# Rongjiehuang/FastDiff

Measured on AMD Instinct MI355X. Metric: real-time factor (audio-sec/wall-sec), N=4 reverse steps, 80x864 mel, higher is better.
Workload: dtype f32 results; 2-piece fp16 operands (22 bit) on fp16 MFMA, fp32 accumulate; GEMM as Winograd F(2,3); exact-fp32 twin; 1 GPU; BASELINE configs[1]: LJSpeech shape, batch=8 x 80x864 mel per GPU, N=4, HIP kernels + hipGraph sampler; batch_per_gpu=8, frames=864, reverse_steps=4, graph=True, weights=random init seed 1234 (no checkpoint offline), world_size=1, gpus_visible=1, oversubscribed=False

## Files before the change

### fastdiff_amd/csrc/fd_kernels_common.h

```cpp
#ifndef FD_KERNELS_COMMON_H
#define FD_KERNELS_COMMON_H
#include "fd_kernels.h"
#include "fd_device.h"

typedef float f32x16 __attribute__((ext_vector_type(16)));

namespace fdk_fast {

__device__ __forceinline__ f32x16 mfma32(float a, float b, f32x16 c)
{
    return __builtin_amdgcn_mfma_f32_32x32x2f32(a, b, c, 0, 0, 0);
}
__device__ __forceinline__ int drow(int r, int hi) { return (r & 3) + 8 * (r >> 2) + 4 * hi; }
__device__ __forceinline__ int opaque(int x)
{
    asm volatile("" : "+v"(x));
    return x;
}
__device__ __forceinline__ float lrelu(float v, float s)
{
    return __builtin_amdgcn_fmed3f(v, v * s, __builtin_inff());
}
__device__ __forceinline__ float f4c(const float4 &v, int r) { return r == 0 ? v.x : (r == 1 ? v.y : (r == 2 ? v.z : v.w)); }

__device__ __forceinline__ int frames_of(const int *lens, int b, int T) { return lens ? lens[b] : T; }

__device__ __forceinline__ bool skip_after_previous_overflow(int *flag)
{
    if (flag[32] == 0) return false;
    if (blockIdx.x == 0 && blockIdx.y == 0 && blockIdx.z == 0 && threadIdx.x == 0) atomicOr(flag, 1);
    return true;
}

constexpr float GX_SCALE = 2048.0f, GX_INV_SCALE = 1.0f / 2048.0f;
constexpr float GX_LIMIT = 32768.0f;
typedef _Float16 f16x8 __attribute__((ext_vector_type(8)));
__device__ __forceinline__ f32x16 mfma_f16(const float4 &a, const float4 &b, f32x16 c)
{
    union { float4 f; f16x8 h; } ua, ub;
    ua.f = a;
    ub.f = b;
    return __builtin_amdgcn_mfma_f32_32x32x16_f16(ua.h, ub.h, c, 0, 0, 0);
}

typedef _Float16 h2_t __attribute__((ext_vector_type(2)));
typedef float f2_t __attribute__((ext_vector_type(2)));

__device__ __forceinline__ void split2(float a, float b, unsigned &hi, unsigned &lo)
{
    const f2_t v = {a, b};
    const h2_t h = __builtin_convertvector(v, h2_t);
    const f2_t r = (v - __builtin_convertvector(h, f2_t)) * GX_SCALE;
    const h2_t l = __builtin_convertvector(r, h2_t);
    hi = __builtin_bit_cast(unsigned, h);
    lo = __builtin_bit_cast(unsigned, l);
}
__device__ __forceinline__ void split8(const float (&v)[8], float4 &hi, float4 &lo)
{
    unsigned h[4], l[4];
#pragma unroll
    for (int i = 0; i < 4; ++i) split2(v[2 * i], v[2 * i + 1], h[i], l[i]);
    hi = make_float4(__uint_as_float(h[0]), __uint_as_float(h[1]), __uint_as_float(h[2]), __uint_as_float(h[3]));
    lo = make_float4(__uint_as_float(l[0]), __uint_as_float(l[1]), __uint_as_float(l[2]), __uint_as_float(l[3]));
}
__device__ __forceinline__ float amax4(float m, const float4 &v) { return fmaxf(fmaxf(m, fmaxf(fabsf(v.x), fabsf(v.y))), fmaxf(fabsf(v.z), fabsf(v.w))); }
__device__ __forceinline__ int h2_off(int row, int slot) { return row * 128 + ((slot ^ ((row >> 1) & 7)) << 4); }
__device__ __forceinline__ void halo_dot(const char *xs, int row, int slot, const float4 &w1f, const float4 &w2f, float &a1, float &a2)
{
    union { float4 f; h2_t h[4]; } x1, x2, w1, w2;
    x1.f = *reinterpret_cast<const float4 *>(xs + h2_off(row, slot));
    x2.f = *reinterpret_cast<const float4 *>(xs + h2_off(row, 4 + slot));
    w1.f = w1f;
    w2.f = w2f;
#pragma unroll
    for (int q = 0; q < 4; ++q) {
        a1 = __builtin_amdgcn_fdot2(w1.h[q], x1.h[q], a1, false);
        a2 = __builtin_amdgcn_fdot2(w1.h[q], x2.h[q], a2, false);
        a2 = __builtin_amdgcn_fdot2(w2.h[q], x1.h[q], a2, false);
    }
}


#ifndef FD_LVC_NT
#define FD_LVC_NT 66
#endif
typedef float lvc_f4 __attribute__((ext_vector_type(4)));
template <int BIT>
__device__ __forceinline__ float4 lvc_ld(const float4 *p)
{
    if constexpr ((FD_LVC_NT & BIT) != 0) {
        const lvc_f4 v = __builtin_nontemporal_load(reinterpret_cast<const lvc_f4 *>(p));
        return make_float4(v.x, v.y, v.z, v.w);
    } else return *p;
}
template <int BIT>
__device__ __forceinline__ void lvc_st(float *p, float v) { if constexpr ((FD_LVC_NT & BIT) != 0) __builtin_nontemporal_store(v, p); else *p = v; }
template <int BIT>
__device__ __forceinline__ void lvc_st(float4 *p, const float4 &v)
{
    if constexpr ((FD_LVC_NT & BIT) != 0) __builtin_nontemporal_store(lvc_f4{v.x, v.y, v.z, v.w}, reinterpret_cast<lvc_f4 *>(p));
    else *p = v;
}

#ifndef FD_LVC_XCD_RUN
#define FD_LVC_XCD_RUN 8
#endif
template <int R = FD_LVC_XCD_RUN>
__device__ __forceinline__ int lvc_tile_of_workgroup()
{
    constexpr int G = 8 * R;
    const int n = blockIdx.x;
    if constexpr (R <= 1) return n;
    const int g0 = (n / G) * G;
    return (g0 + G <= (int)gridDim.x) ? g0 + (n % 8) * R + (n / 8) % R : n;
}

}
#endif
```

### fastdiff_amd/csrc/fd_kernels_dblock.hip

```cpp
#include "fd_kernels_common.h"

namespace fdk_fast {

constexpr int DB_LD = 136;
constexpr int DB_STRIDE = 114;

template <int DIL, bool LRELU>
__device__ __forceinline__ void conv96_tile(f32x16 &acc, const float4 (&wa)[12], const float *in, int ld, int col, int hi)
{
    const int o[3] = {opaque(hi * ld + col - DIL), opaque(hi * ld + col), opaque(hi * ld + col + DIL)};
#pragma unroll
    for (int s = 0; s < 48; ++s) {
        const int tap = s >> 4, c2 = (2 * s) & 31;
        float v = in[o[tap] + c2 * ld];
        if (LRELU) v = lrelu(v, 0.2f);
        acc = mfma32(f4c(wa[s >> 2], s & 3), v, acc);
    }
}

template <int F>
__global__ void __launch_bounds__(256, 2) k_dblock(const float *__restrict__ xin, float *__restrict__ out,
                                                   const float *__restrict__ p0, const float *__restrict__ p1,
                                                   const float *__restrict__ p2, const float *__restrict__ pr,
                                                   const float *__restrict__ b0, const float *__restrict__ b1,
                                                   const float *__restrict__ b2, const float *__restrict__ br, int Lin, int Lo,
                                                   const int *__restrict__ run_if, const int *__restrict__ lens, int per_frame)
{
    __shared__ __attribute__((aligned(16))) float xs[fd::C * DB_LD];
    if (run_if && *run_if == 0) return;
    __shared__ __attribute__((aligned(16))) float hA[fd::C * DB_LD];
    __shared__ __attribute__((aligned(16))) float hB[fd::C * DB_LD];
    const int b = blockIdx.y, tid = threadIdx.x, lane = tid & 63, wave = tid >> 6, l31 = lane & 31, hi = lane >> 5;
    const int pbase = blockIdx.x * DB_STRIDE - 7;
    const int Lob = lens ? lens[b] * per_frame : Lo;
    if (blockIdx.x * DB_STRIDE >= Lob) return;
    {
        constexpr int NK = fd::C * DB_LD / 256;
        float v[NK];
#pragma unroll
        for (int k = 0; k < NK; ++k) {
            const int idx = k * 256 + tid, ci = idx / DB_LD, cc = idx - ci * DB_LD, p = pbase + cc - 4;
            v[k] = (cc >= 4 && cc < 132 && p >= 0 && p < Lob) ? xin[((int64_t)b * fd::C + ci) * Lin + (int64_t)p * F] : 0.0f;
        }
#pragma unroll
        for (int k = 0; k < NK; ++k) {
            const int idx = k * 256 + tid;
            xs[idx] = v[k];
            hA[idx] = 0.0f;
            hB[idx] = 0.0f;
        }
    }
    __syncthreads();
    const int c = wave * 32 + l31;
    const int p = pbase + c;
    const bool inside = (p >= 0 && p < Lob);
    float4 wa[12];
    f32x16 acc;
#pragma unroll
    for (int i = 0; i < 12; ++i) wa[i] = reinterpret_cast<const float4 *>(p0)[i * 64 + lane];
#pragma unroll
    for (int r = 0; r < 16; ++r) acc[r] = b0[drow(r, hi)];
    conv96_tile<1, true>(acc, wa, xs, DB_LD, 4 + c, hi);
#pragma unroll
    for (int r = 0; r < 16; ++r) hA[drow(r, hi) * DB_LD + 4 + c] = inside ? acc[r] : 0.0f;
    __syncthreads();
#pragma unroll
    for (int i = 0; i < 12; ++i) wa[i] = reinterpret_cast<const float4 *>(p1)[i * 64 + lane];
#pragma unroll
    for (int r = 0; r < 16; ++r) acc[r] = b1[drow(r, hi)];
    conv96_tile<2, true>(acc, wa, hA, DB_LD, 4 + c, hi);
#pragma unroll
    for (int r = 0; r < 16; ++r) hB[drow(r, hi) * DB_LD + 4 + c] = inside ? acc[r] : 0.0f;
    __syncthreads();
#pragma unroll
    for (int i = 0; i < 12; ++i) wa[i] = reinterpret_cast<const float4 *>(p2)[i * 64 + lane];
#pragma unroll
    for (int r = 0; r < 16; ++r) acc[r] = b2[drow(r, hi)] + br[drow(r, hi)];
    conv96_tile<4, true>(acc, wa, hB, DB_LD, 4 + c, hi);
    {
        float4 wr[4];
#pragma unroll
        for (int i = 0; i < 4; ++i) wr[i] = reinterpret_cast<const float4 *>(pr)[i * 64 + lane];
#pragma unroll
        for (int s = 0; s < 16; ++s) acc = mfma32(f4c(wr[s >> 2], s & 3), xs[(2 * s + hi) * DB_LD + 4 + c], acc);
    }
    if (inside && c >= 7 && c < 7 + DB_STRIDE) {
#pragma unroll
        for (int r = 0; r < 16; ++r) out[((int64_t)b * fd::C + drow(r, hi)) * Lo + p] = acc[r];
    }
}

constexpr int DBH_ROWS = 136;

template <int DIL>
__device__ __forceinline__ void conv96_h2(f32x16 &ah, f32x16 &al, const float4 (&wa)[2][6], const char *img, int c, int hi)
{
    int off[3][2][2];
#pragma unroll
    for (int tap = 0; tap < 3; ++tap)
#pragma unroll
        for (int p = 0; p < 2; ++p)
#pragma unroll
            for (int c2 = 0; c2 < 2; ++c2) off[tap][p][c2] = h2_off(4 + c + (tap - 1) * DIL, p * 4 + c2 * 2 + hi);
#pragma unroll
    for (int kg = 0; kg < 6; ++kg) {
        const float4 b1 = *reinterpret_cast<const float4 *>(img + off[kg >> 1][0][kg & 1]);
        const float4 b2 = *reinterpret_cast<const float4 *>(img + off[kg >> 1][1][kg & 1]);
        ah = mfma_f16(wa[0][kg], b1, ah);
        al = mfma_f16(wa[0][kg], b2, al);
        al = mfma_f16(wa[1][kg], b1, al);
    }
}
__device__ __forceinline__ void store_act_h2(char *img, const f32x16 &ah, const f32x16 &al, int c, int hi, bool inside, float &mx)
{
    const int row = 4 + c;
#pragma unroll
    for (int j = 0; j < 4; ++j) {
        float v[4];
#pragma unroll
        for (int i = 0; i < 4; ++i) {
            v[i] = inside ? lrelu(fmaf(al[4 * j + i], GX_INV_SCALE, ah[4 * j + i]), 0.2f) : 0.0f;
            mx = fmaxf(mx, fabsf(v[i]));
        }
        uint2 ph, pl;
        split2(v[0], v[1], ph.x, pl.x);
        split2(v[2], v[3], ph.y, pl.y);
        *reinterpret_cast<uint2 *>(img + h2_off(row, j) + 8 * hi) = ph;
        *reinterpret_cast<uint2 *>(img + h2_off(row, 4 + j) + 8 * hi) = pl;
    }
}

#ifndef FD_DBLOCK_OCC
#define FD_DBLOCK_OCC 3
#endif
template <int F, bool AUDIO>
__global__ void __launch_bounds__(256, FD_DBLOCK_OCC) k_dblock_h2(const float *__restrict__ xin, float *__restrict__ out,
                                                      const float4 *__restrict__ p0, const float4 *__restrict__ p1,
                                                      const float4 *__restrict__ p2, const float4 *__restrict__ pr,
                                                      const float *__restrict__ b0, const float *__restrict__ b1,
                                                      const float *__restrict__ b2, const float *__restrict__ br, int Lin, int Lo,
                                                      int *__restrict__ range_flag, const int *__restrict__ lens, int per_frame,
                                                      const float *__restrict__ audio, const float *__restrict__ fw,
                                                      const float *__restrict__ fb)
{
    __shared__ __attribute__((aligned(16))) char xl[DBH_ROWS * 128];
    __shared__ __attribute__((aligned(16))) char xr[DBH_ROWS * 128];
    __shared__ __attribute__((aligned(16))) char ha[DBH_ROWS * 128];
    const int b = blockIdx.y, tid = threadIdx.x, lane = tid & 63, wave = tid >> 6, l31 = lane & 31, hi = lane >> 5;
    const int pbase = blockIdx.x * DB_STRIDE - 7;
    const int Lob = lens ? lens[b] * per_frame : Lo;
    if (blockIdx.x * DB_STRIDE >= Lob || skip_after_previous_overflow(range_flag)) return;
    float mx = 0.0f;
    __shared__ float fwl[AUDIO ? 256 : 1];
    if constexpr (AUDIO) {
        fwl[tid] = tid < 224 ? fw[tid] : fb[tid - 224];
        __syncthreads();
    }
    {
        float v[2][8];
#pragma unroll
        for (int k = 0; k < 2; ++k) {
            const int u = k * 256 + tid, cg = u >> 7, cc = u & 127, p = pbase + cc;
            const bool ok = p >= 0 && p < Lob;
            if (AUDIO) {
                const int Lb = Lob * F, t = p * F;
                const float *xa = audio + (int64_t)b * Lin;
                float xv[7];
#pragma unroll
                for (int i = 0; i < 7; ++i) xv[i] = (ok && t - 3 + i >= 0 && t - 3 + i < Lb) ? xa[t - 3 + i] : 0.0f;
                const int o0 = __builtin_amdgcn_readfirstlane(cg) * 8;
#pragma unroll
                for (int c = 0; c < 8; ++c) {
                    float r = fwl[224 + o0 + c];
#pragma unroll
                    for (int i = 0; i < 7; ++i) r += fwl[(o0 + c) * 7 + i] * xv[i];
                    v[k][c] = ok ? r : 0.0f;
                }
            } else {
#pragma unroll
                for (int c = 0; c < 8; ++c) v[k][c] = ok ? xin[((int64_t)b * fd::C + cg * 8 + c) * Lin + (int64_t)p * F] : 0.0f;
            }
        }
        if (tid < 128) {
            const int g = tid >> 4, row = g < 4 ? g : 128 + g, part = tid & 15;
            *reinterpret_cast<uint2 *>(xl + row * 128 + part * 8) = make_uint2(0u, 0u);
            *reinterpret_cast<uint2 *>(xr + row * 128 + part * 8) = make_uint2(0u, 0u);
            *reinterpret_cast<uint2 *>(ha + row * 128 + part * 8) = make_uint2(0u, 0u);
        }
#pragma unroll
        for (int k = 0; k < 2; ++k) {
            const int u = k * 256 + tid, cg = u >> 7, cc = u & 127;
            float a[8];
#pragma unroll
            for (int c = 0; c < 8; ++c) { mx = fmaxf(mx, fabsf(v[k][c])); a[c] = lrelu(v[k][c], 0.2f); }
            float4 ph, pl;
            split8(v[k], ph, pl);
            *reinterpret_cast<float4 *>(xr + h2_off(4 + cc, cg)) = ph;
            *reinterpret_cast<float4 *>(xr + h2_off(4 + cc, 4 + cg)) = pl;
            split8(a, ph, pl);
            *reinterpret_cast<float4 *>(xl + h2_off(4 + cc, cg)) = ph;
            *reinterpret_cast<float4 *>(xl + h2_off(4 + cc, 4 + cg)) = pl;
        }
    }
    __syncthreads();
    const int c = wave * 32 + l31;
    const int p = pbase + c;
    const bool inside = (p >= 0 && p < Lob);
    float4 wa[2][6];
    f32x16 ah, al;
    auto load_w = [&](const float4 *pk) {
#pragma unroll
        for (int q = 0; q < 2; ++q)
#pragma unroll
            for (int kg = 0; kg < 6; ++kg) wa[q][kg] = pk[(q * 6 + kg) * 64 + lane];
    };
    load_w(p0);
#pragma unroll
    for (int r = 0; r < 16; ++r) { ah[r] = b0[drow(r, hi)]; al[r] = 0.0f; }
    conv96_h2<1>(ah, al, wa, xl, c, hi);
    store_act_h2(ha, ah, al, c, hi, inside, mx);
    __syncthreads();
    load_w(p1);
#pragma unroll
    for (int r = 0; r < 16; ++r) { ah[r] = b1[drow(r, hi)]; al[r] = 0.0f; }
    conv96_h2<2>(ah, al, wa, ha, c, hi);
    store_act_h2(xl, ah, al, c, hi, inside, mx);
    __syncthreads();
    load_w(p2);
#pragma unroll
    for (int r = 0; r < 16; ++r) { ah[r] = b2[drow(r, hi)] + br[drow(r, hi)]; al[r] = 0.0f; }
    conv96_h2<4>(ah, al, wa, xl, c, hi);
    {
        float4 wr[2][2];
#pragma unroll
        for (int q = 0; q < 2; ++q)
#pragma unroll
            for (int kg = 0; kg < 2; ++kg) wr[q][kg] = pr[(q * 2 + kg) * 64 + lane];
#pragma unroll
        for (int kg = 0; kg < 2; ++kg) {
            const float4 x1 = *reinterpret_cast<const float4 *>(xr + h2_off(4 + c, kg * 2 + hi));
            const float4 x2 = *reinterpret_cast<const float4 *>(xr + h2_off(4 + c, 4 + kg * 2 + hi));
            ah = mfma_f16(wr[0][kg], x1, ah);
            al = mfma_f16(wr[0][kg], x2, al);
            al = mfma_f16(wr[1][kg], x1, al);
        }
    }
    if (inside && c >= 7 && c < 7 + DB_STRIDE) {
#pragma unroll
        for (int r = 0; r < 16; ++r) out[((int64_t)b * fd::C + drow(r, hi)) * Lo + p] = fmaf(al[r], GX_INV_SCALE, ah[r]);
    }
    if (!(mx < GX_LIMIT)) atomicOr(range_flag, 1);
}

}

namespace fdk {
using namespace fdk_fast;

hipError_t fast_dblock(const Launch &L, int d, int B, int T, const float *audio)
{
    fd_context *c = L.ctx;
    const DevWeights &w = c->w;
    int Lin = T * fd::HOPT;
    for (int i = 0; i < d; ++i) Lin /= fd::down_factor(i);
    const int f = fd::down_factor(d), Lo = Lin / f;
    const dim3 grid((Lo + DB_STRIDE - 1) / DB_STRIDE, B);
    const int *run_if = nullptr;
    const char *n4 = "dblock_f4", *n8 = "dblock_f8";
    const int *lens = L.mode->ragged ? c->ws.lens_dev : nullptr;
    const Pipe pipe = fd_pipe(*L.mode, L.mode->conv_f16 && w.dblock_f16_ok, 13 + d);
    if (pipe != PIPE_F32_ONLY) {
        int *flag = c->ws.range_flag + 13 + d;
        const float4 *q0 = reinterpret_cast<const float4 *>(w.down_h2[d][0]), *q1 = reinterpret_cast<const float4 *>(w.down_h2[d][1]),
                     *q2 = reinterpret_cast<const float4 *>(w.down_h2[d][2]), *q3 = reinterpret_cast<const float4 *>(w.down_h2[d][3]);
        const float *none = nullptr;
        if (f == 4 && d == 0 && audio)
            FD_LAUNCH(L, n4, (k_dblock_h2<4, true>), grid, dim3(256), 0, c->ws.a[d], c->ws.a[d + 1], q0, q1, q2, q3, w.down[d].conv[0].b,
                      w.down[d].conv[1].b, w.down[d].conv[2].b, w.down[d].res.b, Lin, Lo, flag, lens, Lo / T, audio,
                      (const float *)w.first.w, (const float *)w.first.b);
        else if (f == 4)
            FD_LAUNCH(L, n4, (k_dblock_h2<4, false>), grid, dim3(256), 0, c->ws.a[d], c->ws.a[d + 1], q0, q1, q2, q3, w.down[d].conv[0].b,
                      w.down[d].conv[1].b, w.down[d].conv[2].b, w.down[d].res.b, Lin, Lo, flag, lens, Lo / T, none, none, none);
        else
            FD_LAUNCH(L, n8, (k_dblock_h2<8, false>), grid, dim3(256), 0, c->ws.a[d], c->ws.a[d + 1], q0, q1, q2, q3, w.down[d].conv[0].b,
                      w.down[d].conv[1].b, w.down[d].conv[2].b, w.down[d].res.b, Lin, Lo, flag, lens, Lo / T, none, none, none);
        run_if = flag;
        n4 = n8 = "dblock_fp32_fallback";
        if (pipe == PIPE_F16_ONLY) return hipSuccess;
    }
    if (f == 4)
        FD_LAUNCH(L, n4, k_dblock<4>, grid, dim3(256), 0, c->ws.a[d], c->ws.a[d + 1], w.down_pack[d][0], w.down_pack[d][1],
                  w.down_pack[d][2], w.down_pack[d][3], w.down[d].conv[0].b, w.down[d].conv[1].b, w.down[d].conv[2].b,
                  w.down[d].res.b, Lin, Lo, run_if, lens, Lo / T);
    else
        FD_LAUNCH(L, n8, k_dblock<8>, grid, dim3(256), 0, c->ws.a[d], c->ws.a[d + 1], w.down_pack[d][0], w.down_pack[d][1],
                  w.down_pack[d][2], w.down_pack[d][3], w.down[d].conv[0].b, w.down[d].conv[1].b, w.down[d].conv[2].b,
                  w.down[d].res.b, Lin, Lo, run_if, lens, Lo / T);
    return hipSuccess;
}

}
```

### fastdiff_amd/csrc/fd_kernels_kp.hip

```cpp
#include "fd_kernels_common.h"

namespace fdk_fast {

constexpr int KPF_VALID = 48, KPF_LDI = 68, KPF_LDH = 66;

struct KpFrontW {
    const float *in_pack[fd::NBLK], *in_b[fd::NBLK];
    const float *res_pack[fd::NBLK][6], *res_b[fd::NBLK][6];
};

__global__ void __launch_bounds__(256, 2) k_kp_front(const float *__restrict__ mel, float *__restrict__ hout, KpFrontW w,
                                                     const float *__restrict__ noise, const StepParams *params, int sampler,
                                                     int B, int T, const int *__restrict__ run_if, const int *__restrict__ lens)
{
    __shared__ float xin[fd::COND * KPF_LDI];
    if (run_if && *run_if == 0) return;
    __shared__ float h0[fd::HID * KPF_LDH];
    __shared__ float hA[fd::HID * KPF_LDH];
    __shared__ float hB[fd::HID * KPF_LDH];
    const int blk = blockIdx.z, b = blockIdx.y, t0 = blockIdx.x * KPF_VALID;
    const int Tb = frames_of(lens, b, T);
    if (t0 >= Tb) return;
    const int tid = threadIdx.x, lane = tid & 63, wave = tid >> 6, l31 = lane & 31, hi = lane >> 5;
    const int mt = wave & 1, nt = wave >> 1;
    const int step = sampler ? params->step_idx : 0;
    const float *nz = noise + (((int64_t)step * (sampler > 1 ? B / sampler : B) + b) * fd::NBLK + blk) * fd::COND;
    {
        constexpr int TOTAL = fd::COND * KPF_LDI, NK = (TOTAL + 255) / 256;
        float v[NK];
        const float *src = mel + (int64_t)b * fd::COND * T;
#pragma unroll
        for (int k = 0; k < NK; ++k) {
            const int idx = k * 256 + tid, ci = idx / KPF_LDI, cc = idx - ci * KPF_LDI, t = t0 - 10 + cc;
            v[k] = (idx < TOTAL && t >= 0 && t < Tb) ? src[(int64_t)ci * T + t] + nz[ci] : 0.0f;
        }
#pragma unroll
        for (int k = 0; k < NK; ++k) {
            const int idx = k * 256 + tid;
            if (idx < TOTAL) xin[idx] = v[k];
        }
        if (tid < 128) {
            const int row = tid >> 1, col = (tid & 1) ? KPF_LDH - 1 : 0;
            h0[row * KPF_LDH + col] = 0.0f; hA[row * KPF_LDH + col] = 0.0f; hB[row * KPF_LDH + col] = 0.0f;
        }
    }
    __syncthreads();
    const int c = nt * 32 + l31;
    const int t = t0 - 8 + c;
    const bool inside = (t >= 0 && t < Tb);
    {
        const float4 *pa = reinterpret_cast<const float4 *>(w.in_pack[blk]) + (int64_t)mt * 50 * 64 + lane;
        f32x16 acc;
#pragma unroll
        for (int r = 0; r < 16; ++r) acc[r] = w.in_b[blk][mt * 32 + drow(r, hi)];
#pragma unroll 5
        for (int s4 = 0; s4 < 50; ++s4) {
            const float4 a4 = pa[s4 * 64];
#pragma unroll
            for (int r = 0; r < 4; ++r) {
                const int kk = 8 * s4 + 2 * r, tap = kk / fd::COND, ci = kk % fd::COND + hi;
                acc = mfma32(f4c(a4, r), xin[ci * KPF_LDI + c + tap], acc);
            }
        }
#pragma unroll
        for (int r = 0; r < 16; ++r) h0[(mt * 32 + drow(r, hi)) * KPF_LDH + c + 1] = inside ? lrelu(acc[r], 0.1f) : 0.0f;
    }
    __syncthreads();
    const float *src = h0;
#pragma unroll 1
    for (int l = 0; l < 6; ++l) {
        float *dst = (l & 1) ? hB : hA;
        const float4 *pa = reinterpret_cast<const float4 *>(w.res_pack[blk][l]) + (int64_t)mt * 24 * 64 + lane;
        float4 wa[24];
#pragma unroll
        for (int i = 0; i < 24; ++i) wa[i] = pa[i * 64];
        f32x16 acc;
#pragma unroll
        for (int r = 0; r < 16; ++r) acc[r] = w.res_b[blk][l][mt * 32 + drow(r, hi)];
#pragma unroll
        for (int s = 0; s < 96; ++s) {
            const int tap = s >> 5, ci = ((2 * s) & 63) + hi;
            acc = mfma32(f4c(wa[s >> 2], s & 3), src[ci * KPF_LDH + c + tap], acc);
        }
        if (l < 5) {
#pragma unroll
            for (int r = 0; r < 16; ++r) dst[(mt * 32 + drow(r, hi)) * KPF_LDH + c + 1] = inside ? lrelu(acc[r], 0.1f) : 0.0f;
            __syncthreads();
            src = dst;
        } else if (inside && c >= 8 && c < 8 + KPF_VALID) {
#pragma unroll
            for (int r = 0; r < 16; ++r) {
                const int o = mt * 32 + drow(r, hi);
                hout[(((int64_t)blk * B + b) * fd::HID + o) * T + t] = lrelu(acc[r], 0.1f) + h0[o * KPF_LDH + c + 1];
            }
        }
    }
}

constexpr int KPF_XROW = 336;

struct KpFrontW2 {
    const float4 *in_pack[fd::NBLK];
    const float *in_b[fd::NBLK];
    const float4 *res_pack[fd::NBLK][6];
    const float *res_b[fd::NBLK][6];
};

__device__ __forceinline__ int kpf_off(int row, int slot) { return row * 256 + ((slot ^ (row & 15)) << 4); }

__global__ void __launch_bounds__(256, 2) k_kp_front_h2(const float *__restrict__ mel, float *__restrict__ hout, char *__restrict__ himg,
                                                        KpFrontW2 w, const float *__restrict__ noise, const StepParams *params, int sampler,
                                                        int B, int T, int R, int *__restrict__ range_flags, const int *__restrict__ lens)
{
    __shared__ __attribute__((aligned(16))) char xin[68 * KPF_XROW];
    __shared__ __attribute__((aligned(16))) char hA[66 * 256];
    __shared__ __attribute__((aligned(16))) char hB[66 * 256];
    const int blk = blockIdx.z, b = blockIdx.y, t0 = blockIdx.x * KPF_VALID;
    const int Tb = frames_of(lens, b, T);
    if (range_flags[32 + 19] | range_flags[32]) {
        if (blockIdx.x == 0 && blockIdx.y == 0 && blockIdx.z == 0 && threadIdx.x == 0) { atomicOr(range_flags + 19, 1); atomicOr(range_flags, 1); }
        return;
    }
    if (t0 > Tb) return;
    const int tid = threadIdx.x, lane = tid & 63, wave = tid >> 6, l31 = lane & 31, hi = lane >> 5;
    const int mt = wave & 1, nt = wave >> 1;
    const int step = sampler ? params->step_idx : 0;
    const float *nz = noise + (((int64_t)step * (sampler > 1 ? B / sampler : B) + b) * fd::NBLK + blk) * fd::COND;
    float mx = 0.0f;
    {
        const float *src = mel + (int64_t)b * fd::COND * T;
        float v[3][8];
#pragma unroll
        for (int k = 0; k < 3; ++k) {
            const int u = k * 256 + tid, cg = u / 68, cc = u - cg * 68, t = t0 - 10 + cc;
            const bool ok = u < 680 && t >= 0 && t < Tb;
#pragma unroll
            for (int c = 0; c < 8; ++c) v[k][c] = ok ? src[(int64_t)(cg * 8 + c) * T + t] + nz[cg * 8 + c] : 0.0f;
        }
#pragma unroll
        for (int k = 0; k < 3; ++k) {
            const int u = k * 256 + tid, cg = u / 68, cc = u - cg * 68;
            if (u < 680) {
#pragma unroll
                for (int c = 0; c < 8; ++c) mx = fmaxf(mx, fabsf(v[k][c]));
                float4 ph, pl;
                split8(v[k], ph, pl);
                *reinterpret_cast<float4 *>(xin + cc * KPF_XROW + cg * 16) = ph;
                *reinterpret_cast<float4 *>(xin + cc * KPF_XROW + 160 + cg * 16) = pl;
            }
        }
        if (tid < 64) {
            const int row = (tid & 32) ? 65 : 0, part = tid & 15;
            char *img = (tid & 16) ? hB : hA;
            *reinterpret_cast<float4 *>(img + row * 256 + part * 16) = make_float4(0.f, 0.f, 0.f, 0.f);
        }
    }
    __syncthreads();
    const int c = nt * 32 + l31;
    const int t = t0 - 8 + c;
    const bool inside = (t >= 0 && t < Tb);
    float h0v[16];
    auto store_act = [&](char *img, const f32x16 &ah, const f32x16 &al, float *keep) {
        const int row = c + 1;
#pragma unroll
        for (int j = 0; j < 4; ++j) {
            float v[4];
#pragma unroll
            for (int i = 0; i < 4; ++i) {
                v[i] = inside ? lrelu(fmaf(al[4 * j + i], GX_INV_SCALE, ah[4 * j + i]), 0.1f) : 0.0f;
                mx = fmaxf(mx, fabsf(v[i]));
                if (keep) keep[4 * j + i] = v[i];
            }
            uint2 ph, pl;
            split2(v[0], v[1], ph.x, pl.x);
            split2(v[2], v[3], ph.y, pl.y);
            *reinterpret_cast<uint2 *>(img + kpf_off(row, mt * 4 + j) + 8 * hi) = ph;
            *reinterpret_cast<uint2 *>(img + kpf_off(row, 8 + mt * 4 + j) + 8 * hi) = pl;
        }
    };
    {
        const float4 *pa = w.in_pack[blk] + (int64_t)mt * 2 * 25 * 64 + lane;
        f32x16 ah, al;
#pragma unroll
        for (int r = 0; r < 16; ++r) { ah[r] = w.in_b[blk][mt * 32 + drow(r, hi)]; al[r] = 0.0f; }
        const char *xb = xin + c * KPF_XROW + hi * 16;
#pragma unroll 5
        for (int kg = 0; kg < 25; ++kg) {
            const float4 w1 = pa[kg * 64], w2 = pa[(25 + kg) * 64];
            const int tap = (16 * kg) / fd::COND, o = ((16 * kg) % fd::COND) / 8;
            const float4 b1 = *reinterpret_cast<const float4 *>(xb + tap * KPF_XROW + o * 16);
            const float4 b2 = *reinterpret_cast<const float4 *>(xb + tap * KPF_XROW + 160 + o * 16);
            ah = mfma_f16(w1, b1, ah);
            al = mfma_f16(w1, b2, al);
            al = mfma_f16(w2, b1, al);
        }
        store_act(hA, ah, al, h0v);
    }
    __syncthreads();
    int off[3][2][4];
#pragma unroll
    for (int tap = 0; tap < 3; ++tap)
#pragma unroll
        for (int p = 0; p < 2; ++p)
#pragma unroll
            for (int k4 = 0; k4 < 4; ++k4) off[tap][p][k4] = kpf_off(c + tap, p * 8 + k4 * 2 + hi);
    float4 wa[2][12];
    auto load_w = [&](int l) {
        const float4 *pa = w.res_pack[blk][l] + (int64_t)mt * 2 * 12 * 64 + lane;
#pragma unroll
        for (int p = 0; p < 2; ++p)
#pragma unroll
            for (int kg = 0; kg < 12; ++kg) wa[p][kg] = pa[(p * 12 + kg) * 64];
    };
    load_w(0);
#pragma unroll 1
    for (int l = 0; l < 6; ++l) {
        const char *src = (l & 1) ? hB : hA;
        char *dst = (l & 1) ? hA : hB;
        f32x16 ah, al;
#pragma unroll
        for (int r = 0; r < 16; ++r) { ah[r] = w.res_b[blk][l][mt * 32 + drow(r, hi)]; al[r] = 0.0f; }
#pragma unroll
        for (int kg = 0; kg < 12; ++kg) {
            const float4 b1 = *reinterpret_cast<const float4 *>(src + off[kg >> 2][0][kg & 3]);
            const float4 b2 = *reinterpret_cast<const float4 *>(src + off[kg >> 2][1][kg & 3]);
            ah = mfma_f16(wa[0][kg], b1, ah);
            al = mfma_f16(wa[0][kg], b2, al);
            al = mfma_f16(wa[1][kg], b1, al);
        }
        __builtin_amdgcn_sched_barrier(0);
        if (l < 5) load_w(l + 1);
        __builtin_amdgcn_sched_barrier(0);
        if (l < 5) {
            store_act(dst, ah, al, nullptr);
            __syncthreads();
        } else if (t >= 0 && t < T && c >= 8 && c < 8 + KPF_VALID) {
            char *irow = himg + (((int64_t)blk * B + b) * R + (t + 1)) * 256;
            const int sw = (t + 1) & 15;
#pragma unroll
            for (int j = 0; j < 4; ++j) {
                float v[4];
#pragma unroll
                for (int i = 0; i < 4; ++i) {
                    const int r = 4 * j + i;
                    v[i] = inside ? lrelu(fmaf(al[r], GX_INV_SCALE, ah[r]), 0.1f) + h0v[r] : 0.0f;
                    mx = fmaxf(mx, fabsf(v[i]));
                    hout[(((int64_t)blk * B + b) * fd::HID + mt * 32 + drow(r, hi)) * T + t] = v[i];
                }
                if (himg) {
                    uint2 ph, pl;
                    split2(v[0], v[1], ph.x, pl.x);
                    split2(v[2], v[3], ph.y, pl.y);
                    *reinterpret_cast<uint2 *>(irow + (((mt * 4 + j) ^ sw) << 4) + 8 * hi) = ph;
                    *reinterpret_cast<uint2 *>(irow + (((8 + mt * 4 + j) ^ sw) << 4) + 8 * hi) = pl;
                }
            }
        }
    }
    if (himg) {
        char *ib = himg + ((int64_t)blk * B + b) * R * 256;
        if (blockIdx.x == 0 && tid < 16) *reinterpret_cast<float4 *>(ib + tid * 16) = make_float4(0.f, 0.f, 0.f, 0.f);
        if (blockIdx.x == gridDim.x - 1)
            for (int e = tid; e < (R - 1 - T) * 16; e += 256) *reinterpret_cast<float4 *>(ib + (T + 1) * 256 + e * 16) = make_float4(0.f, 0.f, 0.f, 0.f);
    }
    if (!(mx < GX_LIMIT)) { atomicOr(range_flags + 19, 1); atomicOr(range_flags, 1); }
}

constexpr int GEMM_CT = 4;
constexpr int GEMM_LDH = GEMM_CT * 32 + 4;
constexpr int GEMM_NCOLS = GEMM_CT * 32 + 2;
constexpr int GEMM_NK = (fd::HID * GEMM_NCOLS + 255) / 256;

#ifdef FD_GEMM_TIMING
__device__ long long fd_gdbg[64 * 4 * 4];
#endif

__global__ void __launch_bounds__(256, 2) k_kp_gemm(const float *__restrict__ h , float *__restrict__ kpack,
                                                    const float *g0, const float *g1, const float *g2, const float *gb0,
                                                    const float *gb1, const float *gb2, int B, int T, int chunks_per_utt,
                                                    int chunk_tiles, int n_items, const int *__restrict__ run_if, const int *__restrict__ lens)
{
    __shared__ float hs[2][fd::HID * GEMM_LDH];
    if (run_if && *run_if == 0) return;
    const int tid = threadIdx.x, lane = tid & 63, wave = tid >> 6, l31 = lane & 31, hi = lane >> 5;
    constexpr int XG = fd::KREC / 128;
    const int ny = B * chunks_per_utt;
    const int i0 = (int)((int64_t)blockIdx.x * n_items / gridDim.x), i1 = (int)((int64_t)(blockIdx.x + 1) * n_items / gridDim.x);
    if (i0 >= i1) return;

    struct Item { int blk, xg, b, t_begin; };
    auto decode = [&](int id) {
        Item it;
        it.blk = id / (XG * ny);
        const int rem = id - it.blk * (XG * ny);
        it.xg = rem / ny;
        const int yy = rem - it.xg * ny;
        it.b = yy / chunks_per_utt;
        it.t_begin = (yy - it.b * chunks_per_utt) * chunk_tiles * 32;
        return it;
    };
    float v[33];
    const int scol = tid & 127, srow = tid >> 7;
#define FD_GEMM_FETCH(it)                                                                                              \
    do {                                                                                                               \
        const float *hb__ = h + (((int64_t)(it).blk * B + (it).b) * fd::HID + srow) * T + ((it).t_begin - 1);          \
        const bool ok__ = ((it).t_begin - 1 + scol) >= 0 && ((it).t_begin - 1 + scol) < frames_of(lens, (it).b, T);    \
        _Pragma("unroll") for (int j = 0; j < 32; ++j) v[j] = ok__ ? hb__[(int64_t)(2 * j) * T + scol] : 0.0f;         \
        const int t2__ = (it).t_begin + 127 + (tid & 1);               \
        v[32] = (tid < 128 && t2__ < frames_of(lens, (it).b, T)) ? hb__[(int64_t)((tid >> 1) - srow) * T + 128 + (tid & 1)] : 0.0f;                \
    } while (0)
#define FD_GEMM_COMMIT(bufi)                                                                                           \
    do {                                                                                                               \
        float *hd__ = hs[bufi] + srow * GEMM_LDH + scol;                                                               \
        _Pragma("unroll") for (int j = 0; j < 32; ++j) hd__[2 * j * GEMM_LDH] = v[j];                                   \
        if (tid < 128) hs[bufi][(tid >> 1) * GEMM_LDH + 128 + (tid & 1)] = v[32];                                       \
    } while (0)

    Item cur = decode(i0);
    FD_GEMM_FETCH(cur);
    FD_GEMM_COMMIT(0);
    __syncthreads();
    float4 wb[24];
    float bias = 0.0f;
    int have_blk = -1, have_xg = -1, buf = 0;
#pragma unroll 1
    for (int i = i0; i < i1; ++i) {
        if (cur.blk != have_blk || cur.xg != have_xg) {
            const float *gp = cur.blk == 0 ? g0 : (cur.blk == 1 ? g1 : g2);
            const float *gb = cur.blk == 0 ? gb0 : (cur.blk == 1 ? gb1 : gb2);
            const int ptile = cur.xg * 4 + wave;
#pragma unroll
            for (int k = 0; k < 24; ++k) wb[k] = reinterpret_cast<const float4 *>(gp)[((int64_t)ptile * 24 + k) * 64 + lane];
            bias = gb[ptile * 32 + l31];
            have_blk = cur.blk; have_xg = cur.xg;
        }
        Item nxt = cur;
        const bool more = (i + 1 < i1);
        if (more) { nxt = decode(i + 1); FD_GEMM_FETCH(nxt); }
        const int Tb = frames_of(lens, cur.b, T);
        const int n_frames = min(Tb - cur.t_begin, chunk_tiles * 32);
        const int n_tiles = (n_frames + 31) >> 5;
        float *kout = kpack + ((int64_t)cur.blk * B + cur.b) * T * fd::KREC + (cur.xg * 4 + wave) * 32 + l31;
#pragma unroll 1
        for (int tile = 0; tile < n_tiles; ++tile) {
            f32x16 acc;
#pragma unroll
            for (int r = 0; r < 16; ++r) acc[r] = bias;
            const int hc = hi * GEMM_LDH + l31 + tile * 32;
            const int ho3[3] = {opaque(hc), opaque(hc + 1), opaque(hc + 2)};
#pragma unroll
            for (int s = 0; s < 96; ++s) {
                const int tap = s >> 5, c2 = (2 * s) & 63;
                acc = mfma32(hs[buf][ho3[tap] + c2 * GEMM_LDH], f4c(wb[s >> 2], s & 3), acc);
            }
            const int t0 = cur.t_begin + tile * 32;
            const unsigned base = (unsigned)(t0 + 4 * hi) * (unsigned)fd::KREC;
#ifdef FD_GX_NO_STORE
            if (acc[0] != 12345.678f) continue;
#endif
            if (t0 + 32 <= Tb) {
#pragma unroll
                for (int r = 0; r < 16; ++r) kout[base + (unsigned)(((r & 3) + 8 * (r >> 2)) * fd::KREC)] = acc[r];
            } else {
#pragma unroll
                for (int r = 0; r < 16; ++r)
                    if (t0 + drow(r, hi) < Tb) kout[base + (unsigned)(((r & 3) + 8 * (r >> 2)) * fd::KREC)] = acc[r];
            }
        }
        if (more) FD_GEMM_COMMIT(buf ^ 1);
        __syncthreads();
        buf ^= 1;
        cur = nxt;
    }
}

constexpr int GX_ROWS = GX_CT * 32 + 2;
constexpr int GX_WINB = GX_ROWS * GX_ROWB;
constexpr int GX_NDMA = (GX_WINB + 4095) / 4096;
constexpr int GX_BUFB = GX_NDMA * 4096;
#ifndef FD_GX_STORE_AUX
#define FD_GX_STORE_AUX 2
#endif


__global__ void __launch_bounds__(256) k_h_split(const float *__restrict__ h, unsigned *__restrict__ hx, int *__restrict__ range_flag,
                                                 int B, int T, int R, const int *__restrict__ lens)
{
    const int bb = blockIdx.y;
    const int e = blockIdx.x * 256 + threadIdx.x, cp = e / R, row = e - cp * R;
    if (cp >= 32) return;
    if (range_flag[32] != 0) {
        if (e == 0 && bb == 0) atomicOr(range_flag, 1);
        return;
    }
    const int t = row - 1;
    const bool ok = t >= 0 && t < frames_of(lens, bb % B, T);
    const float *hb = h + (int64_t)bb * fd::HID * T;
    const float a = ok ? hb[(int64_t)(2 * cp) * T + t] : 0.0f, b2 = ok ? hb[(int64_t)(2 * cp + 1) * T + t] : 0.0f;
    if (!(fmaxf(fabsf(a), fabsf(b2)) < GX_LIMIT)) atomicOr(range_flag, 1);
    const _Float16 a1 = (_Float16)a, b1 = (_Float16)b2;
    const _Float16 a2 = (_Float16)((a - (float)a1) * GX_SCALE), b3 = (_Float16)((b2 - (float)b1) * GX_SCALE);
    union { _Float16 h[2]; unsigned u; } p1, p2;
    p1.h[0] = a1; p1.h[1] = b1;
    p2.h[0] = a2; p2.h[1] = b3;
    unsigned *dst = hx + ((int64_t)bb * R + row) * 64 + (cp & 3);
    const unsigned sw = (unsigned)row & 15u, slot = (unsigned)cp >> 2;
    dst[((slot ^ sw) << 2)] = p1.u;
    dst[(((slot + 8u) ^ sw) << 2)] = p2.u;
}

typedef __attribute__((address_space(3))) void *lds_ptr_t;

struct GxItem { int blk, xg, b, chunk; };

struct GxWalk {
    static constexpr int XG = fd::KREC / 128;
    int B, chunks, ny, n_wg, w, q, base, r0, r1;
    int n_mine, left0;
    __device__ __forceinline__ GxWalk(int B_, int chunks_per_utt, int n_items, int n_wg_, int w_)
// ... 502 lines not shown
```

Measured before the change: 9962 x real-time.

## Prefetch conv weights and biases ahead of barriers in dblock and KP front kernels

Restructures the dblock and KP front kernels so the next layer's weight loads are issued before the store/sync of the current layer. Biases are staged once into shared memory and read as float4 instead of per-row global loads. Audio taps for the first conv are loaded before the shared-memory barrier, and the KP input-conv weights are double-buffered in groups of five. Also adds compile-time-gated timestamp instrumentation that is off by default. The aim is to hide global-load latency behind MFMA work, at the cost of more registers and possible occupancy pressure.

```diff
diff --git a/fastdiff_amd/csrc/fd_kernels_common.h b/fastdiff_amd/csrc/fd_kernels_common.h
--- a/fastdiff_amd/csrc/fd_kernels_common.h
+++ b/fastdiff_amd/csrc/fd_kernels_common.h
@@ -115,5 +115,21 @@
     return (g0 + G <= (int)gridDim.x) ? g0 + (n % 8) * R + (n / 8) % R : n;
 }
 
+#ifdef FD_CHAIN_STAMP
+constexpr int CH_NWG = 4096, CH_NST = 16;
+#define CH_DECL long long ch_t[CH_NST] = {}
+#define CH_STAMP(k) do { __builtin_amdgcn_sched_barrier(0); asm volatile("s_memrealtime %0\n\ts_waitcnt lgkmcnt(0)" : "=s"(ch_t[k]) :: "memory"); \
+                         __builtin_amdgcn_sched_barrier(0); } while (0)
+#define CH_LAP_FROM(j) do { ch_t[CH_NST - 1] = ch_t[j]; } while (0)
+#define CH_LAP(k) do { const long long l__ = ch_t[CH_NST - 1]; CH_STAMP(CH_NST - 1); ch_t[k] += ch_t[CH_NST - 1] - l__; } while (0)
+#define CH_FLUSH(buf, wg) do { if (threadIdx.x == 0 && (wg) < CH_NWG) { _Pragma("unroll") for (int i__ = 0; i__ < CH_NST; ++i__) (buf)[(wg) * CH_NST + i__] = ch_t[i__]; } } while (0)
+#else
+#define CH_DECL do { } while (0)
+#define CH_STAMP(k) do { } while (0)
+#define CH_LAP_FROM(j) do { } while (0)
+#define CH_LAP(k) do { } while (0)
+#define CH_FLUSH(buf, wg) do { } while (0)
+#endif
+
 }
 #endif
diff --git a/fastdiff_amd/csrc/fd_kernels_dblock.hip b/fastdiff_amd/csrc/fd_kernels_dblock.hip
--- a/fastdiff_amd/csrc/fd_kernels_dblock.hip
+++ b/fastdiff_amd/csrc/fd_kernels_dblock.hip
@@ -133,6 +133,9 @@
 #ifndef FD_DBLOCK_OCC
 #define FD_DBLOCK_OCC 3
 #endif
+#ifdef FD_CHAIN_STAMP
+__device__ long long fd_chain_dbg_dblock[CH_NWG * CH_NST];
+#endif
 template <int F, bool AUDIO>
 __global__ void __launch_bounds__(256, FD_DBLOCK_OCC) k_dblock_h2(const float *__restrict__ xin, float *__restrict__ out,
                                                       const float4 *__restrict__ p0, const float4 *__restrict__ p1,
@@ -150,36 +153,63 @@
     const int pbase = blockIdx.x * DB_STRIDE - 7;
     const int Lob = lens ? lens[b] * per_frame : Lo;
     if (blockIdx.x * DB_STRIDE >= Lob || skip_after_previous_overflow(range_flag)) return;
+    CH_DECL;
+    CH_STAMP(0);
     float mx = 0.0f;
+    float4 wa[2][6], wr[2][2];
+    auto load_w = [&](const float4 *pk) {
+#pragma unroll
+        for (int q = 0; q < 2; ++q)
+#pragma unroll
+            for (int kg = 0; kg < 6; ++kg) wa[q][kg] = pk[(q * 6 + kg) * 64 + lane];
+    };
+    __shared__ __attribute__((aligned(16))) float bl[96];
+    float bv = 0.0f;
+    if (tid < 96) bv = tid < 32 ? b0[tid] : (tid < 64 ? b1[tid - 32] : b2[tid - 64] + br[tid - 64]);
     __shared__ float fwl[AUDIO ? 256 : 1];
+    float xv[AUDIO ? 2 : 1][7];
     if constexpr (AUDIO) {
-        fwl[tid] = tid < 224 ? fw[tid] : fb[tid - 224];
+        const float fv = tid < 224 ? fw[tid] : fb[tid - 224];
+        const float *xa = audio + (int64_t)b * Lin;
+#pragma unroll
+        for (int k = 0; k < 2; ++k) {
+            const int p = pbase + ((k * 256 + tid) & 127), Lb = Lob * F, t = p * F;
+            const bool ok = p >= 0 && p < Lob;
+#pragma unroll
+            for (int i = 0; i < 7; ++i) xv[k][i] = (ok && t - 3 + i >= 0 && t - 3 + i < Lb) ? xa[t - 3 + i] : 0.0f;
+        }
+        __builtin_amdgcn_sched_barrier(0);
+        fwl[tid] = fv;
+        if (tid < 96) bl[tid] = bv;
         __syncthreads();
-    }
+    } else {
+        if (tid < 96) bl[tid] = bv;
+    }
+    CH_STAMP(1);
     {
         float v[2][8];
 #pragma unroll
         for (int k = 0; k < 2; ++k) {
             const int u = k * 256 + tid, cg = u >> 7, cc = u & 127, p = pbase + cc;
             const bool ok = p >= 0 && p < Lob;
-            if (AUDIO) {
-                const int Lb = Lob * F, t = p * F;
-                const float *xa = audio + (int64_t)b * Lin;
-                float xv[7];
-#pragma unroll
-                for (int i = 0; i < 7; ++i) xv[i] = (ok && t - 3 + i >= 0 && t - 3 + i < Lb) ? xa[t - 3 + i] : 0.0f;
+            if constexpr (AUDIO) {
                 const int o0 = __builtin_amdgcn_readfirstlane(cg) * 8;
 #pragma unroll
                 for (int c = 0; c < 8; ++c) {
                     float r = fwl[224 + o0 + c];
 #pragma unroll
-                    for (int i = 0; i < 7; ++i) r += fwl[(o0 + c) * 7 + i] * xv[i];
+                    for (int i = 0; i < 7; ++i) r += fwl[(o0 + c) * 7 + i] * xv[k][i];
                     v[k][c] = ok ? r : 0.0f;
                 }
             } else {
 #pragma unroll
                 for (int c = 0; c < 8; ++c) v[k][c] = ok ? xin[((int64_t)b * fd::C + cg * 8 + c) * Lin + (int64_t)p * F] : 0.0f;
             }
+        }
+        if constexpr (!AUDIO) {
+            __builtin_amdgcn_sched_barrier(0);
+            load_w(p0);
+            __builtin_amdgcn_sched_barrier(0);
         }
         if (tid < 128) {
             const int g = tid >> 4, row = g < 4 ? g : 128 + g, part = tid & 15;
@@ -202,57 +232,79 @@
             *reinterpret_cast<float4 *>(xl + h2_off(4 + cc, 4 + cg)) = pl;
         }
     }
-    __syncthreads();
+    if constexpr (AUDIO) {
+        __builtin_amdgcn_sched_barrier(0);
+        load_w(p0);
+        __builtin_amdgcn_sched_barrier(0);
+    }
+    CH_STAMP(2);
+    __syncthreads();
+    CH_STAMP(3);
     const int c = wave * 32 + l31;
     const int p = pbase + c;
     const bool inside = (p >= 0 && p < Lob);
-    float4 wa[2][6];
     f32x16 ah, al;
-    auto load_w = [&](const float4 *pk) {
-#pragma unroll
-        for (int q = 0; q < 2; ++q)
-#pragma unroll
-            for (int kg = 0; kg < 6; ++kg) wa[q][kg] = pk[(q * 6 + kg) * 64 + lane];
+    auto load_b = [&](int l) {
+#pragma unroll
+        for (int j = 0; j < 4; ++j) {
+            const float4 t4 = *reinterpret_cast<const float4 *>(bl + l * 32 + 8 * j + 4 * hi);
+            ah[4 * j] = t4.x; ah[4 * j + 1] = t4.y; ah[4 * j + 2] = t4.z; ah[4 * j + 3] = t4.w;
+        }
+#pragma unroll
+        for (int r = 0; r < 16; ++r) al[r] = 0.0f;
     };
-    load_w(p0);
-#pragma unroll
-    for (int r = 0; r < 16; ++r) { ah[r] = b0[drow(r, hi)]; al[r] = 0.0f; }
+    load_b(0);
     conv96_h2<1>(ah, al, wa, xl, c, hi);
+    __builtin_amdgcn_sched_barrier(0);
+    load_w(p1);
+#pragma unroll
+    for (int q = 0; q < 2; ++q)
+#pragma unroll
+        for (int kg = 0; kg < 2; ++kg) wr[q][kg] = pr[(q * 2 + kg) * 64 + lane];
+    __builtin_amdgcn_sched_barrier(0);
+    CH_STAMP(4);
     store_act_h2(ha, ah, al, c, hi, inside, mx);
     __syncthreads();
-    load_w(p1);
-#pragma unroll
-    for (int r = 0; r < 16; ++r) { ah[r] = b1[drow(r, hi)]; al[r] = 0.0f; }
+    CH_STAMP(5);
+    load_b(1);
     conv96_h2<2>(ah, al, wa, ha, c, hi);
+    __builtin_amdgcn_sched_barrier(0);
+    load_w(p2);
+    __builtin_amdgcn_sched_barrier(0);
+    CH_STAMP(6);
     store_act_h2(xl, ah, al, c, hi, inside, mx);
     __syncthreads();
-    load_w(p2);
-#pragma unroll
-    for (int r = 0; r < 16; ++r) { ah[r] = b2[drow(r, hi)] + br[drow(r, hi)]; al[r] = 0.0f; }
+    CH_STAMP(7);
+    load_b(2);
     conv96_h2<4>(ah, al, wa, xl, c, hi);
-    {
-        float4 wr[2][2];
-#pragma unroll
-        for (int q = 0; q < 2; ++q)
-#pragma unroll
-            for (int kg = 0; kg < 2; ++kg) wr[q][kg] = pr[(q * 2 + kg) * 64 + lane];
-#pragma unroll
-        for (int kg = 0; kg < 2; ++kg) {
-            const float4 x1 = *reinterpret_cast<const float4 *>(xr + h2_off(4 + c, kg * 2 + hi));
-            const float4 x2 = *reinterpret_cast<const float4 *>(xr + h2_off(4 + c, 4 + kg * 2 + hi));
-            ah = mfma_f16(wr[0][kg], x1, ah);
-            al = mfma_f16(wr[0][kg], x2, al);
-            al = mfma_f16(wr[1][kg], x1, al);
-        }
-    }
+    CH_STAMP(8);
+#pragma unroll
+    for (int kg = 0; kg < 2; ++kg) {
+        const float4 x1 = *reinterpret_cast<const float4 *>(xr + h2_off(4 + c, kg * 2 + hi));
+        const float4 x2 = *reinterpret_cast<const float4 *>(xr + h2_off(4 + c, 4 + kg * 2 + hi));
+        ah = mfma_f16(wr[0][kg], x1, ah);
+        al = mfma_f16(wr[0][kg], x2, al);
+        al = mfma_f16(wr[1][kg], x1, al);
+    }
+    CH_STAMP(9);
     if (inside && c >= 7 && c < 7 + DB_STRIDE) {
 #pragma unroll
         for (int r = 0; r < 16; ++r) out[((int64_t)b * fd::C + drow(r, hi)) * Lo + p] = fmaf(al[r], GX_INV_SCALE, ah[r]);
     }
     if (!(mx < GX_LIMIT)) atomicOr(range_flag, 1);
-}
-
-}
+    CH_STAMP(10);
+    if constexpr (AUDIO) CH_FLUSH(fd_chain_dbg_dblock, blockIdx.y * gridDim.x + blockIdx.x);
+}
+
+}
+
+#ifdef FD_CHAIN_STAMP
+extern "C" __attribute__((visibility("default"))) int fd_chain_dbg_read_dblock(long long *out, int n)
+{
+    if (hipDeviceSynchronize() != hipSuccess) return -1;
+    return hipMemcpyFromSymbol(out, HIP_SYMBOL(fdk_fast::fd_chain_dbg_dblock), sizeof(long long) * n) == hipSuccess ? 0 : -1;
+}
+#endif
 
 namespace fdk {
 using namespace fdk_fast;
diff --git a/fastdiff_amd/csrc/fd_kernels_kp.hip b/fastdiff_amd/csrc/fd_kernels_kp.hip
--- a/fastdiff_amd/csrc/fd_kernels_kp.hip
+++ b/fastdiff_amd/csrc/fd_kernels_kp.hip
@@ -107,6 +107,9 @@
 };
 
 __device__ __forceinline__ int kpf_off(int row, int slot) { return row * 256 + ((slot ^ (row & 15)) << 4); }
+#ifdef FD_CHAIN_STAMP
+__device__ long long fd_chain_dbg_kp[CH_NWG * CH_NST];
+#endif
 
 __global__ void __launch_bounds__(256, 2) k_kp_front_h2(const float *__restrict__ mel, float *__restrict__ hout, char *__restrict__ himg,
                                                         KpFrontW2 w, const float *__restrict__ noise, const StepParams *params, int sampler,
@@ -122,6 +125,8 @@
         return;
     }
     if (t0 > Tb) return;
+    CH_DECL;
+    CH_STAMP(0);
     const int tid = threadIdx.x, lane = tid & 63, wave = tid >> 6, l31 = lane & 31, hi = lane >> 5;
     const int mt = wave & 1, nt = wave >> 1;
     const int step = sampler ? params->step_idx : 0;
@@ -155,7 +160,24 @@
             *reinterpret_cast<float4 *>(img + row * 256 + part * 16) = make_float4(0.f, 0.f, 0.f, 0.f);
         }
     }
+    __shared__ __attribute__((aligned(16))) float kb[7 * fd::HID];
+    {
+        const int wu = __builtin_amdgcn_readfirstlane(wave);
+        kb[wu * 64 + lane] = (wu == 0 ? w.in_b[blk] : w.res_b[blk][wu - 1])[lane];
+        if (wu < 3) kb[(wu + 4) * 64 + lane] = w.res_b[blk][wu + 3][lane];
+    }
+    const float4 *pa0 = w.in_pack[blk] + (int64_t)mt * 2 * 25 * 64 + lane;
+    float4 w0[2][2][5];
+    auto load_w0 = [&](int set, int g) {
+#pragma unroll
+        for (int i = 0; i < 5; ++i) { w0[set][0][i] = pa0[(5 * g + i) * 64]; w0[set][1][i] = pa0[(25 + 5 * g + i) * 64]; }
+    };
+    __builtin_amdgcn_sched_barrier(0);
+    load_w0(0, 0);
+    __builtin_amdgcn_sched_barrier(0);
+    CH_STAMP(1);
     __syncthreads();
+    CH_STAMP(2);
     const int c = nt * 32 + l31;
     const int t = t0 - 8 + c;
     const bool inside = (t >= 0 && t < Tb);
@@ -178,32 +200,15 @@
             *reinterpret_cast<uint2 *>(img + kpf_off(row, 8 + mt * 4 + j) + 8 * hi) = pl;
         }
     };
-    {
-        const float4 *pa = w.in_pack[blk] + (int64_t)mt * 2 * 25 * 64 + lane;
-        f32x16 ah, al;
-#pragma unroll
-        for (int r = 0; r < 16; ++r) { ah[r] = w.in_b[blk][mt * 32 + drow(r, hi)]; al[r] = 0.0f; }
-        const char *xb = xin + c * KPF_XROW + hi * 16;
-#pragma unroll 5
-        for (int kg = 0; kg < 25; ++kg) {
-            const float4 w1 = pa[kg * 64], w2 = pa[(25 + kg) * 64];
-            const int tap = (16 * kg) / fd::COND, o = ((16 * kg) % fd::COND) / 8;
-            const float4 b1 = *reinterpret_cast<const float4 *>(xb + tap * KPF_XROW + o * 16);
-            const float4 b2 = *reinterpret_cast<const float4 *>(xb + tap * KPF_XROW + 160 + o * 16);
-            ah = mfma_f16(w1, b1, ah);
-            al = mfma_f16(w1, b2, al);
-            al = mfma_f16(w2, b1, al);
-        }
-        store_act(hA, ah, al, h0v);
-    }
-    __syncthreads();
-    int off[3][2][4];
-#pragma unroll
-    for (int tap = 0; tap < 3; ++tap)
-#pragma unroll
-        for (int p = 0; p < 2; ++p)
-#pragma unroll
-            for (int k4 = 0; k4 < 4; ++k4) off[tap][p][k4] = kpf_off(c + tap, p * 8 + k4 * 2 + hi);
+    auto load_b = [&](int l, f32x16 &ah, f32x16 &al) {
+#pragma unroll
+        for (int j = 0; j < 4; ++j) {
+            const float4 t4 = *reinterpret_cast<const float4 *>(kb + l * 64 + mt * 32 + 8 * j + 4 * hi);
+            ah[4 * j] = t4.x; ah[4 * j + 1] = t4.y; ah[4 * j + 2] = t4.z; ah[4 * j + 3] = t4.w;
+        }
+#pragma unroll
+        for (int r = 0; r < 16; ++r) al[r] = 0.0f;
+    };
     float4 wa[2][12];
     auto load_w = [&](int l) {
         const float4 *pa = w.res_pack[blk][l] + (int64_t)mt * 2 * 12 * 64 + lane;
@@ -212,14 +217,50 @@
 #pragma unroll
             for (int kg = 0; kg < 12; ++kg) wa[p][kg] = pa[(p * 12 + kg) * 64];
     };
-    load_w(0);
+    {
+        f32x16 ah, al;
+        load_b(0, ah, al);
+        const char *xb = xin + c * KPF_XROW + hi * 16;
+#pragma unroll
+        for (int g = 0; g < 5; ++g) {
+            if (g < 4) {
+                __builtin_amdgcn_sched_barrier(0);
+                load_w0((g + 1) & 1, g + 1);
+                __builtin_amdgcn_sched_barrier(0);
+            }
+#pragma unroll
+            for (int i = 0; i < 5; ++i) {
+                const int kg = 5 * g + i;
+                const int tap = (16 * kg) / fd::COND, o = ((16 * kg) % fd::COND) / 8;
+                const float4 b1 = *reinterpret_cast<const float4 *>(xb + tap * KPF_XROW + o * 16);
+                const float4 b2 = *reinterpret_cast<const float4 *>(xb + tap * KPF_XROW + 160 + o * 16);
+                ah = mfma_f16(w0[g & 1][0][i], b1, ah);
+                al = mfma_f16(w0[g & 1][0][i], b2, al);
+                al = mfma_f16(w0[g & 1][1][i], b1, al);
+            }
+        }
+        __builtin_amdgcn_sched_barrier(0);
+        load_w(0);
+        __builtin_amdgcn_sched_barrier(0);
+        CH_STAMP(3);
+        store_act(hA, ah, al, h0v);
+    }
+    __syncthreads();
+    CH_STAMP(4);
+    int off[3][2][4];
+#pragma unroll
+    for (int tap = 0; tap < 3; ++tap)
+#pragma unroll
+        for (int p = 0; p < 2; ++p)
+#pragma unroll
+            for (int k4 = 0; k4 < 4; ++k4) off[tap][p][k4] = kpf_off(c + tap, p * 8 + k4 * 2 + hi);
+    CH_LAP_FROM(4);
 #pragma unroll 1
     for (int l = 0; l < 6; ++l) {
         const char *src = (l & 1) ? hB : hA;
         char *dst = (l & 1) ? hA : hB;
         f32x16 ah, al;
-#pragma unroll
-        for (int r = 0; r < 16; ++r) { ah[r] = w.res_b[blk][l][mt * 32 + drow(r, hi)]; al[r] = 0.0f; }
+        load_b(l + 1, ah, al);
 #pragma unroll
         for (int kg = 0; kg < 12; ++kg) {
             const float4 b1 = *reinterpret_cast<const float4 *>(src + off[kg >> 2][0][kg & 3]);
@@ -231,9 +272,11 @@
         __builtin_amdgcn_sched_barrier(0);
         if (l < 5) load_w(l + 1);
         __builtin_amdgcn_sched_barrier(0);
+        CH_LAP(5);
         if (l < 5) {
             store_act(dst, ah, al, nullptr);
             __syncthreads();
+            CH_LAP(6);
         } else if (t >= 0 && t < T && c >= 8 && c < 8 + KPF_VALID) {
             char *irow = himg + (((int64_t)blk * B + b) * R + (t + 1)) * 256;
             const int sw = (t + 1) & 15;
@@ -264,7 +307,19 @@
             for (int e = tid; e < (R - 1 - T) * 16; e += 256) *reinterpret_cast<float4 *>(ib + (T + 1) * 256 + e * 16) = make_float4(0.f, 0.f, 0.f, 0.f);
     }
     if (!(mx < GX_LIMIT)) { atomicOr(range_flags + 19, 1); atomicOr(range_flags, 1); }
-}
+    CH_STAMP(7);
+    CH_FLUSH(fd_chain_dbg_kp, (blockIdx.z * gridDim.y + blockIdx.y) * gridDim.x + blockIdx.x);
+}
+
+#ifdef FD_CHAIN_STAMP
+}
+extern "C" __attribute__((visibility("default"))) int fd_chain_dbg_read_kp(long long *out, int n)
+{
+    if (hipDeviceSynchronize() != hipSuccess) return -1;
+    return hipMemcpyFromSymbol(out, HIP_SYMBOL(fdk_fast::fd_chain_dbg_kp), sizeof(long long) * n) == hipSuccess ? 0 : -1;
+}
+namespace fdk_fast {
+#endif
 
 constexpr int GEMM_CT = 4;
 constexpr int GEMM_LDH = GEMM_CT * 32 + 4;
```

Result: no change. 10060 x real-time (median of 6 runs) (+1.0%).
